# dominikh/jello

Hardware: AMD Instinct MI355X
Metric: Mpixels/sec fine-raster + paths/sec, 100k-path 4096^2 scene (higher is better)
Workload: dtype f32

## Files before the change

jello_amd/csrc/kernels_flatten.hip:

```cpp
#include <hip/hip_runtime.h>
__shared__ double fl_atan_tab[9];
#define JD_ATAN_TAB_LDS fl_atan_tab
#include "kcommon.h"
#define FF_INLINE __device__ __forceinline__
#include "flatten_fast.h"

using namespace jk;
using namespace jd;

namespace {

struct CubicParams { float th0, th1, chord_len, err; };
struct EulerParams { float th0, th1, k0, k1, ch; };
struct CubicPoints { V2 p0, p1, p2, p3; };
struct PointDeriv { V2 point, deriv; };
struct PathTagData { uint32_t tag_byte; MonoidK<5> monoid; };

#define DERIV_THRESH 1e-6f
#define DERIV_THRESH_SQUARED (DERIV_THRESH * DERIV_THRESH)
#define DERIV_EPS 1e-6f
#define SUBDIV_LIMIT (1.0f / 65536.0f)
#define K1_THRESH 1e-3f
#define DIST_THRESH 1e-3f
#define TANGENT_THRESH 1e-6f

#define FL_INVALID 0xffffffffu
#define FL_INFO_PIECE 0x80000000u
#define FL_INFO_DIRECT 0x40000000u
#ifndef FL_REFILL_LANES
#define FL_REFILL_LANES 32u
#endif

#define FL_MAX_REGIONS 8u
#define FL_MAX_GRAB 51200u
struct FlTemp {
    uint2* sinfo;
    uint4* recs;
    uint32_t* ctr;
    uint32_t K, R;
};
#define FL_CTR_CURSOR 512u
#define FL_CUR_STRIDE 64u
template <int KIND>
JD uint32_t fl_grab(const FlTemp& T, uint32_t home, uint32_t n, bool& failed) {
    uint32_t p = wave_bump(T.ctr + FL_CTR_CURSOR + FL_CUR_STRIDE * home + (KIND ? 32u : 0u), n);
    if (__builtin_expect(p <= T.R && n <= T.R - p, 1)) return home * T.R + p;
    failed = true;
    uint32_t region = home;
    for (uint32_t tries = 1u;; tries++) {
        if (KIND == 0 && p < T.R)
            for (uint32_t i = p; i < T.R; i++) T.sinfo[(size_t)region * T.R + i] = make_uint2(0u, 0u);
        if (p >= T.R) atomicSub(T.ctr + FL_CTR_CURSOR + FL_CUR_STRIDE * region + (KIND ? 32u : 0u), n);
        if (tries >= T.K) return FL_INVALID;
        region = region + 1u == T.K ? 0u : region + 1u;
        p = atomicAdd(T.ctr + FL_CTR_CURSOR + FL_CUR_STRIDE * region + (KIND ? 32u : 0u), n);
        if (p <= T.R && n <= T.R - p) return region * T.R + p;
    }
}
JD uint32_t fl_next_home(const FlTemp& T, uint32_t home, int kind) {
    uint32_t region = home;
    for (uint32_t tries = 0u; tries < T.K; tries++) {
        const uint32_t cur = __hip_atomic_load(T.ctr + FL_CTR_CURSOR + FL_CUR_STRIDE * region + (kind ? 32u : 0u), __ATOMIC_RELAXED, __HIP_MEMORY_SCOPE_AGENT);
        if (cur < T.R) return region;
        region = region + 1u == T.K ? 0u : region + 1u;
    }
    return home;
}

template <bool EMIT>
struct Out {
    const JlConfig* cfg;
    FlTemp T;
    uint32_t home_s, home_r;
    bool failed_s, failed_r;
    uint32_t slot;
    uint32_t cursor;
    uint32_t a_first, a_spos, a_rpos;

    JD uint32_t alloc(uint32_t n) {
        uint32_t first = cursor;
        cursor += n;
        if (EMIT) {
            a_first = first;
            a_spos = fl_grab<0>(T, home_s, n, failed_s);
            a_rpos = fl_grab<1>(T, home_r, n, failed_r);
        }
        return first;
    }
// ... 487 lines not shown
    }
}


JD V2 read_f32_point(const Scene& s, uint32_t ix) {
    uint32_t b = s.cfg->layout.pathdata_base + ix;
    return v2(u2f(s.scene.rd(b)), u2f(s.scene.rd(b + 1u)));
}
JD V2 read_i16_point(const Scene& s, uint32_t ix) {
    uint32_t raw = s.scene.rd(s.cfg->layout.pathdata_base + ix);
    float x = (float)((int32_t)(raw << 16) >> 16);
    float y = (float)((int32_t)raw >> 16);
    return v2(x, y);
}
JD PathTagData compute_tag_monoid(const Scene& s, uint32_t ix) {
    uint32_t tag_word = s.scene.rd(s.cfg->layout.pathtag_base + (ix >> 2));
    uint32_t shift = (ix & 3u) * 8u;
    MonoidK<5> tm = reduce_tag(tag_word & ((1u << shift) - 1u));
    JlTagMonoid pm = s.tag_monoids.rd(ix >> 2);
    tm.v[0] += pm.trans_ix; tm.v[1] += pm.pathseg_ix; tm.v[2] += pm.pathseg_offset; tm.v[3] += pm.style_ix; tm.v[4] += pm.path_ix;
    PathTagData r;
    r.tag_byte = (tag_word >> shift) & 0xffu;
    tm.v[0] -= 1u;
    tm.v[3] -= 2u;
    r.monoid = tm;
    return r;
}
JD CubicPoints read_path_segment(const Scene& s, const PathTagData& tag, bool is_stroke) {
    V2 p0 = v2(0, 0), p1 = v2(0, 0), p2 = v2(0, 0), p3 = v2(0, 0);
    uint32_t seg_type = tag.tag_byte & 3u;
    uint32_t pathseg_offset = tag.monoid.v[2];
    bool is_stroke_cap_marker = is_stroke && (tag.tag_byte & JL_PATH_TAG_SUBPATH_END) != 0u;
    bool is_open = seg_type == JL_PATH_TAG_QUADTO;
    if ((tag.tag_byte & JL_PATH_TAG_F32) != 0u) {
        p0 = read_f32_point(s, pathseg_offset);
        p1 = read_f32_point(s, pathseg_offset + 2u);
        if (seg_type >= JL_PATH_TAG_QUADTO) {
            p2 = read_f32_point(s, pathseg_offset + 4u);
            if (seg_type == JL_PATH_TAG_CUBICTO) p3 = read_f32_point(s, pathseg_offset + 6u);
        }
    } else {
        p0 = read_i16_point(s, pathseg_offset);
        p1 = read_i16_point(s, pathseg_offset + 1u);
        if (seg_type >= JL_PATH_TAG_QUADTO) {
            p2 = read_i16_point(s, pathseg_offset + 2u);
            if (seg_type == JL_PATH_TAG_CUBICTO) p3 = read_i16_point(s, pathseg_offset + 3u);
        }
    }
    if (is_stroke_cap_marker && is_open) {
        p0 = p1;
        p1 = p2;
        seg_type = JL_PATH_TAG_LINETO;
    }
    const float THIRD = (float)(1.0 / 3.0);
    if (seg_type == JL_PATH_TAG_LINETO) {
        p3 = p1;
        p2 = vmix(p3, p0, THIRD);
        p1 = vmix(p0, p3, THIRD);
    } else if (seg_type == JL_PATH_TAG_QUADTO) {
        p3 = p2;
        p2 = vmix(p1, p2, THIRD);
        p1 = vmix(p1, p0, THIRD);
    }
    CubicPoints r;
    r.p0 = p0; r.p1 = p1; r.p2 = p2; r.p3 = p3;
    return r;
}

struct Seg {
    PathTagData tag;
    uint32_t style_flags;
    bool is_stroke;
};

JD Seg load_seg(const Scene& s, uint32_t ix) {
    Seg r;
    r.tag = compute_tag_monoid(s, ix);
    r.style_flags = s.scene.rd(s.cfg->layout.style_base + r.tag.monoid.v[3]);
    r.is_stroke = (r.style_flags & JL_STYLE_FLAGS_STYLE) != 0u;
    return r;
}

#define FL_CTR_LIGHT 256u
#define FL_CTR_DEAL (FL_CTR_CURSOR + FL_CUR_STRIDE * FL_MAX_REGIONS)
#define FL_DEAL_GROUPS 256u
#define FL_DEAL_STRIDE 16u
#define FL_CTR_WORDS (FL_CTR_DEAL + FL_DEAL_STRIDE * FL_DEAL_GROUPS)
#ifndef PSC_BLOCKS
#define PSC_BLOCKS 2u
#endif
template <int SCAN>
__global__ __launch_bounds__(JL_WG) void k_flatten_classify(const JlConfig* __restrict__ cfg, Buf<uint32_t> scene, Buf<JlTagMonoid> reduced,
                                                                 Buf<JlTagMonoid> tag_monoids, uint32_t n_blocks, Buf<JlPathBbox> path_bboxes,
                                                                 uint32_t* __restrict__ list, uint32_t* __restrict__ counters, uint32_t cap,
                                                                 uint32_t n_tags, uint32_t* __restrict__ counts, uint32_t absorb,
                                                                 uint32_t* __restrict__ bump_words) {
    __shared__ uint32_t sh[20];
    __shared__ uint32_t sh_base[2];
    if (absorb & JH_ABSORB_BBOX_CLEAR) {
        const uint32_t n_clear = umin_(cfg->layout.n_path, path_bboxes.n);
        for (uint32_t i = blockIdx.x * JL_WG + threadIdx.x; i < n_clear; i += gridDim.x * JL_WG) {
            path_bboxes.p[i].x0 = 0x7fffffff;
            path_bboxes.p[i].y0 = 0x7fffffff;
            path_bboxes.p[i].x1 = (int32_t)0x80000000;
            path_bboxes.p[i].y1 = (int32_t)0x80000000;
        }
    }
    if ((absorb & JH_ABSORB_BUMP_CLEAR) && blockIdx.x == 0u && threadIdx.x < 8u) bump_words[threadIdx.x] = 0u;
    uint32_t nh[PSC_BLOCKS][4], nl[PSC_BLOCKS][4];
    uint32_t eh[PSC_BLOCKS], el[PSC_BLOCKS];
    uint32_t wg_h = 0u, wg_l = 0u;
#pragma unroll
    for (uint32_t blk = 0; blk < PSC_BLOCKS; blk++) {
        const uint32_t block = blockIdx.x * PSC_BLOCKS + blk;
        eh[blk] = 0u; el[blk] = 0u;
#pragma unroll
        for (uint32_t k = 0; k < 4u; k++) { nh[blk][k] = 0u; nl[blk][k] = 0u; }
        if (block >= n_blocks) continue;
        const uint32_t word_ix = block * JL_WG + threadIdx.x;
        const uint32_t tag_word = scene.rd(cfg->layout.pathtag_base + word_ix);
        MonoidK<5> pm;
        if (SCAN != 0) {
            MonoidK<5> prefix;
            if (SCAN == 1) prefix = parent_prefix(reduced, block, sh); else prefix = load_tm(reduced, block);
            MonoidK<5> tot5;
            if (SCAN == 1) __syncthreads();
            const MonoidK<5> ex = block_excl_scan_monoid<5>(reduce_tag(tag_word), sh, &tot5);
            pm = monoid_add(prefix, ex);
            if (tag_monoids.ok(word_ix)) {
                store_tm(&tag_monoids.p[word_ix], pm);
            } else {
#pragma unroll
                for (int i = 0; i < 5; i++) pm.v[i] = 0u;
            }
            __syncthreads();
        } else {
            pm = load_tm(tag_monoids, word_ix);
        }
        const uint32_t ix0 = word_ix * 4u;
        for (uint32_t q = 0u; q < 12u; q++) {
            const uint32_t sl = ix0 * 3u + q;
            if (sl < cap) counts[sl] = 0u;
        }
        uint32_t th = 0u, tl = 0u;
#pragma unroll
        for (uint32_t k = 0; k < 4u; k++) {
            const uint32_t ix = ix0 + k;
            if (ix >= n_tags) continue;
            const MonoidK<5> tm = monoid_add(pm, reduce_tag(tag_word & ((1u << (k * 8u)) - 1u)));
            const uint32_t tag_byte = (tag_word >> (k * 8u)) & 0xffu;
            const uint32_t style_flags = scene.rd(cfg->layout.style_base + tm.v[3] - 2u);
            const bool is_stroke = (style_flags & JL_STYLE_FLAGS_STYLE) != 0u;
            const uint32_t path_ix = tm.v[4];
            if ((tag_byte & JL_PATH_TAG_PATH) != 0u && path_bboxes.ok(path_ix)) {
                path_bboxes.p[path_ix].draw_flags = ((style_flags & JL_STYLE_FLAGS_FILL) == 0u) ? 0u : 1u;
                path_bboxes.p[path_ix].trans_ix = tm.v[0] - 1u;
            }
            const uint32_t seg_type = tag_byte & JL_PATH_TAG_SEG_TYPE;
            const bool curved = seg_type != JL_PATH_TAG_LINETO;
            if (seg_type != 0u) {
                if (!is_stroke) {
                    if (curved) nh[blk][k] = 1u; else nl[blk][k] = 1u;
                } else if ((tag_byte & JL_PATH_TAG_SUBPATH_END) != 0u) {
                    if (curved) nl[blk][k] = 1u;
                } else {
                    if (curved) { nh[blk][k] = 2u; nl[blk][k] = 1u; } else { nl[blk][k] = 3u; }
                }
            }
            th += nh[blk][k];
            tl += nl[blk][k];
        }
        MonoidK<2> m, tot;
        m.v[0] = th; m.v[1] = tl;
        const MonoidK<2> e2 = block_excl_scan_monoid<2>(m, sh, &tot);
        eh[blk] = wg_h + e2.v[0];
        el[blk] = wg_l + e2.v[1];
        wg_h += tot.v[0];
        wg_l += tot.v[1];
        __syncthreads();
    }
    if (threadIdx.x == 0) {
        sh_base[0] = wg_h ? atomicAdd(&counters[0], wg_h) : 0u;
        sh_base[1] = wg_l ? atomicAdd(&counters[FL_CTR_LIGHT], wg_l) : 0u;
    }
    __syncthreads();
#pragma unroll
    for (uint32_t blk = 0; blk < PSC_BLOCKS; blk++) {
        const uint32_t ix0 = ((blockIdx.x * PSC_BLOCKS + blk) * JL_WG + threadIdx.x) * 4u;
        uint32_t ph = sh_base[0] + eh[blk], pl = sh_base[1] + el[blk];
#pragma unroll
        for (uint32_t k = 0; k < 4u; k++) {
            const uint32_t ix = ix0 + k;
            uint32_t sub = 0u;
            for (uint32_t q = 0; q < nh[blk][k]; q++, sub++, ph++)
                if (ph < cap) list[ph] = ix * 3u + sub;
            for (uint32_t q = 0; q < nl[blk][k]; q++, sub++, pl++)
                if (pl < cap) list[cap - 1u - pl] = ix * 3u + sub;
        }
    }
}

template <bool EMIT>
JD void run_item(const JlConfig* cfg, const Scene& s, Out<EMIT>& o, uint32_t slot, EulerJob& job, uint32_t& path_ix_out) {
    uint32_t ix = slot / 3u, sub = slot - ix * 3u;
    Seg g = load_seg(s, ix);
    uint32_t path_ix = g.tag.monoid.v[4];
    path_ix_out = path_ix;
    uint32_t style_ix = g.tag.monoid.v[3];
    uint32_t trans_ix = g.tag.monoid.v[0];
    uint32_t style_flags = g.style_flags;
    job.path_ix = path_ix; job.trans_ix = trans_ix;
    Xf transform;
    {
        uint32_t base = cfg->layout.transform_base + trans_ix * 6u;
        transform.m0 = u2f(s.scene.rd(base)); transform.m1 = u2f(s.scene.rd(base + 1u)); transform.m2 = u2f(s.scene.rd(base + 2u));
        transform.m3 = u2f(s.scene.rd(base + 3u)); transform.t0 = u2f(s.scene.rd(base + 4u)); transform.t1 = u2f(s.scene.rd(base + 5u));
    }
    CubicPoints pts = read_path_segment(s, g.tag, g.is_stroke);
    if (g.is_stroke) {
        float linewidth = u2f(s.scene.rd(cfg->layout.style_base + style_ix + 1u));
        float offset = 0.5f * linewidth;
        bool is_stroke_cap_marker = (g.tag.tag_byte & JL_PATH_TAG_SUBPATH_END) != 0u;
        if (is_stroke_cap_marker) {
            V2 tangent = cubic_start_tangent(pts.p0, pts.p1, pts.p2, pts.p3);
            V2 offset_tangent = offset * normalize(tangent);
            V2 n = v2(offset_tangent.y * -1.0f, offset_tangent.x * 1.0f);
            draw_cap<EMIT>(o, path_ix, (style_flags & JL_STYLE_FLAGS_START_CAP_MASK) >> 2, pts.p0, pts.p0 - n, pts.p0 + n, -offset_tangent,
                           transform);
        } else {
            const float TT = TANGENT_THRESH * TANGENT_THRESH;
            V2 tan_prev = cubic_end_tangent(pts.p0, pts.p1, pts.p2, pts.p3);
            if (dot(tan_prev, tan_prev) < TT) tan_prev = v2(TANGENT_THRESH, 0.0f);
            V2 offset_tangent = offset * normalize(tan_prev);
            V2 n_prev = v2(offset_tangent.y * -1.0f, offset_tangent.x * 1.0f);
            if (sub < 2u) {
                V2 tan_start = cubic_start_tangent(pts.p0, pts.p1, pts.p2, pts.p3);
                if (dot(tan_start, tan_start) < TT) tan_start = v2(TANGENT_THRESH, 0.0f);
                V2 n_start = offset * normalize(v2(-tan_start.y, tan_start.x));
                job.valid = true; job.cubic = pts; job.local_to_device = transform;
                if (sub == 0u) { job.offset = offset; job.start_p = pts.p0 + n_start; job.end_p = pts.p3 + n_prev; }
                else { job.offset = -offset; job.start_p = pts.p0 - n_start; job.end_p = pts.p3 - n_prev; }
            } else {
                PathTagData ntag = compute_tag_monoid(s, ix + 1u);
                CubicPoints npts = read_path_segment(s, ntag, true);
                bool n_is_closed = (ntag.tag_byte & JL_PATH_TAG_SEG_TYPE) == JL_PATH_TAG_LINETO;
                bool n_is_marker = (ntag.tag_byte & JL_PATH_TAG_SUBPATH_END) != 0u;
                bool do_join = !n_is_marker || n_is_closed;
                if (do_join) {
                    V2 tan_next = cubic_start_tangent(npts.p0, npts.p1, npts.p2, npts.p3);
                    if (dot(tan_next, tan_next) < TT) tan_next = v2(TANGENT_THRESH, 0.0f);
                    V2 tnn = normalize(tan_next);
                    V2 n_next = v2((offset * tnn.y) * -1.0f, (offset * tnn.x) * 1.0f);
                    draw_join<EMIT>(o, path_ix, style_flags, pts.p3, tan_prev, tan_next, n_prev, n_next, transform);
                } else {
                    draw_cap<EMIT>(o, path_ix, (style_flags & JL_STYLE_FLAGS_END_CAP_MASK), pts.p3, pts.p3 + n_prev, pts.p3 - n_prev, offset_tangent,
                                   transform);
                }
            }
        }
    } else {
        job.valid = true; job.cubic = pts; job.local_to_device = transform;
        job.offset = 0.0f; job.start_p = pts.p0; job.end_p = pts.p3;
    }
}

#ifndef FLQ_STACK
#define FLQ_STACK 448u
#endif
#ifndef FLQ_LEAVES
#define FLQ_LEAVES 640u
#endif
#ifndef FLQ_MAX_LEVEL
#define FLQ_MAX_LEVEL 9u
#endif
struct FlBatch {
    uint32_t jhead[64];
    uint32_t stack[FLQ_STACK];
    uint32_t l_tpos[FLQ_LEAVES];
    uint16_t l_key[FLQ_LEAVES];
    uint16_t l_link[FLQ_LEAVES];
// ... 84 lines not shown
JD CubicParams piece_angles(const NodeEnds& ne) {
    const V2 chord = ne.point - ne.last_p;
    const float chord_squared = dot(chord, chord);
    CubicParams r;
    r.err = 0.0f;
    if (chord_squared < DERIV_THRESH_SQUARED) {
        r.th0 = 0.0f; r.th1 = 0.0f; r.chord_len = DERIV_THRESH;
        return r;
    }
    const V2 q0 = ne.last_q, q1 = ne.deriv;
    const V2 h0 = v2(q0.x * chord.x + q0.y * chord.y, q0.y * chord.x - q0.x * chord.y);
    const V2 h1 = v2(q1.x * chord.x + q1.y * chord.y, q1.x * chord.y - q1.y * chord.x);
    r.th0 = atan2_(h0.y, h0.x);
    r.th1 = atan2_(h1.y, h1.x);
    r.chord_len = sqrt_(chord_squared);
    return r;
}

struct PieceParams {
    EulerParams ep;
    float n, noff, int0, integral;
    uint32_t n_u, robust;
};
JD PieceParams piece_params(const CubicParams& cp, float scale, float offset) {
    const float tol = 0.25f;
    PieceParams r;
    r.ep = es_params_from_angles(cp.th0, cp.th1);
    const EulerParams& ep = r.ep;
    float k0 = ep.k0 - 0.5f * ep.k1;
    float k1 = ep.k1;
    float normalized_offset = offset / cp.chord_len;
    float dist_scaled = normalized_offset * ep.ch;
    float scale_multiplier = sqrt_(0.125f * scale * cp.chord_len / (ep.ch * tol));
    float a = 0.0f, b = 0.0f, integral = 0.0f, int0 = 0.0f, n_frac;
    uint32_t robust = 0u;
    if (abs_(k1) < K1_THRESH) {
        float k = ep.k0;
        n_frac = sqrt_(abs_(k * (k * dist_scaled + 1.0f)));
        robust = 1u;
    } else if (abs_(dist_scaled) < DIST_THRESH) {
        a = k1;
        b = k0;
        int0 = pow_1_5_signed(b);
        float int1 = pow_1_5_signed(a + b);
        integral = int1 - int0;
        n_frac = (float)(2.0 / 3.0) * integral / a;
        robust = 2u;
    } else {
        a = -2.0f * dist_scaled * k1;
        b = -1.0f - 2.0f * dist_scaled * k0;
        int0 = espc_int_approx(b);
        float int1 = espc_int_approx(a + b);
        integral = int1 - int0;
        float k_peak = k0 - k1 * b / a;
        float integrand_peak = sqrt_(abs_(k_peak * (k_peak * dist_scaled + 1.0f)));
        n_frac = integral * integrand_peak / a;
    }
    r.n = clamp_(ceil_(n_frac * scale_multiplier), 1.0f, 100.0f);
    r.n_u = to_u32(r.n);
    r.noff = normalized_offset;
    r.int0 = int0;
    r.integral = integral;
    r.robust = robust;
    return r;
}

#ifdef FL_FAST_CHECK
__device__ uint32_t g_ff_stats[8];
#endif
#ifndef FL_WAVES_PER_EU
#define FL_WAVES_PER_EU 4
#endif
#ifndef FL_BLOCKS_PER_CU
#define FL_BLOCKS_PER_CU 4
#endif
#ifdef FL_TIMING
#define FL_TL_WAVES 8192u
#define FL_TL_BATCHES 15u
#define FL_TL_WORDS (2u + 3u * FL_TL_BATCHES)
__device__ unsigned long long g_fl_timeline[FL_TL_WAVES * FL_TL_WORDS];
#endif
__global__ __launch_bounds__(JL_WG) __attribute__((amdgpu_waves_per_eu(FL_WAVES_PER_EU, FL_WAVES_PER_EU))) void k_flatten_items(const JlConfig* __restrict__ cfg, Buf<uint32_t> scene, Buf<JlTagMonoid> tag_monoids,
                                                         Buf<JlPathBbox> path_bboxes, const uint32_t* __restrict__ list,
                                                         uint32_t* __restrict__ counters, uint32_t cap, uint32_t* __restrict__ counts,
                                                         FlTemp T, uint32_t debug) {
    __shared__ FlBatch sh_batch[JL_WG / 64];
    Scene s;
    s.cfg = cfg; s.scene = scene; s.tag_monoids = tag_monoids;
    uint32_t n_heavy = umin_(counters[0], cap), n_light = umin_(counters[FL_CTR_LIGHT], cap - n_heavy);
    uint32_t n = n_heavy + n_light;
    const uint32_t units_h = n_heavy / 64u + (n_heavy % 64u != 0u ? 1u : 0u);
    const uint32_t units = units_h + n_light / 64u + (n_light % 64u != 0u ? 1u : 0u);
    const uint32_t n_groups = umin_(umax_(gridDim.x / FL_BLOCKS_PER_CU, 1u), FL_DEAL_GROUPS), group = blockIdx.x % n_groups;
    if (group >= units) return;
#ifdef FL_TIMING
    const unsigned long long tl_entry = wall_clock64();
    const uint32_t tl_wave = blockIdx.x * (JL_WG / 64u) + (threadIdx.x >> 6);
    uint32_t tl_n = 0u;
#endif
    atan_tab_fill();
    __syncthreads();
    const uint32_t lane = lane_id();
    FlBatch& B = sh_batch[threadIdx.x >> 6];
    Out<true> o;
    o.cfg = cfg; o.T = T; o.home_s = o.home_r = blockIdx.x % T.K; o.failed_s = o.failed_r = false; o.slot = 0u;
    if ((debug & 1u) != 0u) o.home_s = o.home_r = 0u;
#ifdef FL_SOAK_HOME0
    o.home_s = o.home_r = 0u;
#endif
    o.cursor = 0u; o.a_first = 0u; o.a_spos = 0u; o.a_rpos = 0u;
    for (;;) {
        uint32_t k = 0u;
        if (lane == 0u) k = atomicAdd(&counters[FL_CTR_DEAL + FL_DEAL_STRIDE * group], 1u);
        k = uni(k);
        const uint32_t u = k * n_groups + group;
        if (u >= units) break;
        const bool heavy = u < units_h;
        const uint32_t t_first = heavy ? u * 64u : n_heavy + (u - units_h) * 64u;
        const uint32_t t_end = umin_(t_first + 64u, heavy ? n_heavy : n);
        const uint32_t t = t_first + lane;
#ifdef FL_TIMING
        const unsigned long long tl_start = wall_clock64() | (heavy ? 1ull << 63 : 0ull);
        uint32_t tl_info = 0u;
#define FL_TL_END()                                                                                      \
    do {                                                                                                 \
        if (lane == 0u && tl_wave < FL_TL_WAVES && tl_n < FL_TL_BATCHES) {                               \
            g_fl_timeline[tl_wave * FL_TL_WORDS + 2u + 3u * tl_n] = tl_start;                            \
            g_fl_timeline[tl_wave * FL_TL_WORDS + 3u + 3u * tl_n] = wall_clock64();                      \
            g_fl_timeline[tl_wave * FL_TL_WORDS + 4u + 3u * tl_n] = tl_info;                             \
        }                                                                                                \
        tl_n++;                                                                                          \
    } while (0)
#else
#define FL_TL_END() do {} while (0)
#endif
        if (__builtin_amdgcn_ballot_w64(o.failed_s) != 0ull) { o.home_s = fl_next_home(T, o.home_s, 0); o.failed_s = false; }
        if (__builtin_amdgcn_ballot_w64(o.failed_r) != 0ull) { o.home_r = fl_next_home(T, o.home_r, 1); o.failed_r = false; }
        EulerJob job;
        job.valid = false; job.path_ix = 0u; job.trans_ix = 0u; job.offset = 0.0f;
        job.start_p = v2(0, 0); job.end_p = v2(0, 0);
        job.cubic.p0 = job.cubic.p1 = job.cubic.p2 = job.cubic.p3 = v2(0, 0);
        job.local_to_device = xf_identity();
        uint32_t slot = FL_INVALID;
        if (t < t_end) {
            slot = heavy ? list[t] : list[cap - 1u - (t - n_heavy)];
            o.slot = slot; o.cursor = 0u; o.a_first = 0u; o.a_spos = 0u; o.a_rpos = 0u;
            uint32_t path_ix;
            run_item<true>(cfg, s, o, slot, job, path_ix);
            if (!job.valid) counts[slot] = o.cursor;
        }
        EulerLane e;
        euler_begin(e, job);
        const bool active = job.valid && !e.done;
        if (__builtin_amdgcn_ballot_w64(active) == 0ull) {
            FL_TL_END();
            continue;
        }
        B.jhead[lane] = 0u;
        {
            const uint64_t am = __builtin_amdgcn_ballot_w64(active);
            if (active) B.stack[(uint32_t)__builtin_popcountll(am & ((1ull << lane) - 1ull))] = lane;
            if (lane == 0u) { B.n_stack = (uint32_t)__builtin_popcountll(am); B.n_leaves = 0u; B.bail = 0u; B.n_unsure = 0u; }
        }
        wave_sync();
#ifdef FL_SPLIT_NO_A
        if (lane == 0u) B.n_stack = 0u;
        wave_sync();
#endif
        for (;;) {
#ifdef FL_TIMING
            tl_info += 1u << 16;
#endif
            const uint32_t ns = uni(B.n_stack);
            const uint32_t nu = (uint32_t)__builtin_amdgcn_readfirstlane((int)B.n_unsure);
            if (ns == 0u && nu == 0u) break;
            const bool exact_round = ns == 0u || nu >= 64u;
            const uint32_t take = umin_(exact_round ? nu : ns, 64u);
            const bool has = lane < take;
            const uint32_t node = has ? (exact_round ? B.unsure[nu - 1u - lane] : B.stack[ns - 1u - lane]) : 0u;
            wave_sync();
            const uint32_t j = node & 63u, level = (node >> 6) & 31u, t0_u = node >> 11;
            const V2 jp0 = v2(read_lane_var(e.p0.x, j), read_lane_var(e.p0.y, j)), jp1 = v2(read_lane_var(e.p1.x, j), read_lane_var(e.p1.y, j));
            const V2 jp2 = v2(read_lane_var(e.p2.x, j), read_lane_var(e.p2.y, j)), jp3 = v2(read_lane_var(e.p3.x, j), read_lane_var(e.p3.y, j));
            const float scale = read_lane_var(e.scale, j);
            int kind = ffast::FF_UNSURE;
            if (exact_round) {
                if (has) kind = node_test(jp0, jp1, jp2, jp3, scale, level, t0_u).accept ? ffast::FF_ACCEPT : ffast::FF_REJECT;
            } else if (has) {
                float v_est, delta;
                kind = node_test_fast(jp0, jp1, jp2, jp3, scale, level, t0_u, &v_est, &delta);
#ifdef FL_FAST_CHECK
            }
            if (!exact_round) {
                bool c_unsure = false, c_contra = false, c_viol = false;
                if (has) {
                    float v2_, d2_;
                    const int k2 = node_test_fast(jp0, jp1, jp2, jp3, scale, level, t0_u, &v2_, &d2_);
                    const NodeResult rx = node_test(jp0, jp1, jp2, jp3, scale, level, t0_u);
                    const float vx = rx.cp.err * scale;
                    c_unsure = k2 == ffast::FF_UNSURE;
                    c_contra = (k2 == ffast::FF_ACCEPT && !rx.accept) || (k2 == ffast::FF_REJECT && rx.accept);
                    c_viol = (d2_ > 0.0f && !(abs_(v2_ - vx) <= d2_)) || (d2_ == 0.0f && k2 != ffast::FF_UNSURE && v2_ != 0.0f);
                }
                const uint32_t n0 = (uint32_t)__builtin_popcountll(__builtin_amdgcn_ballot_w64(has));
                const uint32_t n1 = (uint32_t)__builtin_popcountll(__builtin_amdgcn_ballot_w64(c_unsure));
                const uint32_t n2 = (uint32_t)__builtin_popcountll(__builtin_amdgcn_ballot_w64(c_contra));
                const uint32_t n3 = (uint32_t)__builtin_popcountll(__builtin_amdgcn_ballot_w64(c_viol));
                if (lane == 0u) {
                    atomicAdd(&g_ff_stats[0], n0);
                    if (n1) atomicAdd(&g_ff_stats[1], n1);
                    if (n2) atomicAdd(&g_ff_stats[2], n2);
                    if (n3) atomicAdd(&g_ff_stats[3], n3);
                }
#endif
            }
            const bool acc = has && kind == ffast::FF_ACCEPT, rej = has && kind == ffast::FF_REJECT, uns = has && kind == ffast::FF_UNSURE;
            const uint64_t accm = __builtin_amdgcn_ballot_w64(acc), rejm = __builtin_amdgcn_ballot_w64(rej), unsm = __builtin_amdgcn_ballot_w64(uns);
            const uint32_t n_acc = (uint32_t)__builtin_popcountll(accm), n_rej = (uint32_t)__builtin_popcountll(rejm);
            const uint32_t n_uns = (uint32_t)__builtin_popcountll(unsm);
            const uint32_t nl = uni(B.n_leaves);
            const uint32_t ns_left = exact_round ? ns : ns - take, nu_left = exact_round ? nu - take : nu;
            const bool too_deep = __builtin_amdgcn_ballot_w64(rej && level + 1u > FLQ_MAX_LEVEL) != 0ull;
            if (too_deep || ns_left + 2u * n_rej > FLQ_STACK || nl + n_acc > FLQ_LEAVES) {
                if (lane == 0u) B.bail = 1u;
                wave_sync();
                break;
            }
            const uint64_t below = (1ull << lane) - 1ull;
// ... 358 lines not shown
        const int32_t c = imax_(x1, dpp_move<CTRL, ROWS>(x1, x1)), d = imax_(y1, dpp_move<CTRL, ROWS>(y1, y1)); \
        if (take) { x0 = a; y0 = b; x1 = c; y1 = d; }                                        \
    }
            FB_SEG_STEP(JK_DPP_ROW_SHR(1), 0xf) FB_SEG_STEP(JK_DPP_ROW_SHR(2), 0xf) FB_SEG_STEP(JK_DPP_ROW_SHR(4), 0xf)
            FB_SEG_STEP(JK_DPP_ROW_SHR(8), 0xf) FB_SEG_STEP(JK_DPP_ROW_BCAST15, 0xa) FB_SEG_STEP(JK_DPP_ROW_BCAST31, 0xc)
#undef FB_SEG_STEP
            if (pix == c_path) {
                x0 = imin_(x0, cx0); y0 = imin_(y0, cy0); x1 = imax_(x1, cx1); y1 = imax_(y1, cy1);
            }
            const uint32_t pix_next = lane_next(pix, pix);
            if (valid && !skipped && pix_next != pix) fb_merge(path_bboxes, pix, x0, y0, x1, y1, pix == p_shared);
            c_path = (uint32_t)__builtin_amdgcn_readlane((int)pix, 63);
            cx0 = __builtin_amdgcn_readlane(x0, 63); cy0 = __builtin_amdgcn_readlane(y0, 63);
            cx1 = __builtin_amdgcn_readlane(x1, 63); cy1 = __builtin_amdgcn_readlane(y1, 63);
            if (ext) break;
        }
        if (c_path != FB_NONE && lane == 0u) fb_merge(path_bboxes, c_path, cx0, cy0, cx1, cy1, c_path == p_shared);
    }
}

}

#ifdef FL_FAST_CHECK
extern "C" int jh_debug_flatten_fast_stats(uint32_t* out8, int reset) {
    if (hipDeviceSynchronize() != hipSuccess) return -1;
    if (out8 && hipMemcpyFromSymbol(out8, HIP_SYMBOL(g_ff_stats), 8 * sizeof(uint32_t)) != hipSuccess) return -1;
    if (reset) {
        const uint32_t z[8] = {0, 0, 0, 0, 0, 0, 0, 0};
        if (hipMemcpyToSymbol(HIP_SYMBOL(g_ff_stats), z, sizeof z) != hipSuccess) return -1;
    }
    return 0;
}
#endif

#ifdef FL_TIMING
extern "C" int jh_debug_flatten_timeline(unsigned long long* out, uint32_t n_words, int reset, uint32_t* dims3) {
    if (hipDeviceSynchronize() != hipSuccess) return -1;
    if (dims3) {
        int dev = 0, khz = 0;
        if (hipGetDevice(&dev) != hipSuccess || hipDeviceGetAttribute(&khz, hipDeviceAttributeWallClockRate, dev) != hipSuccess) return -1;
        dims3[0] = FL_TL_WAVES; dims3[1] = FL_TL_WORDS; dims3[2] = (uint32_t)khz;
    }
    if (out) {
        if (n_words > FL_TL_WAVES * FL_TL_WORDS) return -1;
        if (hipMemcpyFromSymbol(out, HIP_SYMBOL(g_fl_timeline), (size_t)n_words * 8u) != hipSuccess) return -1;
    }
    if (reset) {
        void* p = nullptr;
        if (hipGetSymbolAddress(&p, HIP_SYMBOL(g_fl_timeline)) != hipSuccess) return -1;
        if (hipMemset(p, 0, sizeof(unsigned long long) * FL_TL_WAVES * FL_TL_WORDS) != hipSuccess) return -1;
    }
    return 0;
}
#endif

JhResult jh_launch_flatten(const JhLaunch& L) {
    if (L.gx == 0) return JH_L_OK;
    uint32_t n_tags = L.gx * JL_WG;
    uint64_t n_slots64 = (uint64_t)n_tags * 3;
    if (n_slots64 > 0xfffffff0ull) return JH_L_BAD_BINDINGS;
    uint32_t n_slots = (uint32_t)n_slots64;
    auto cfg = L.ptr<const JlConfig>(FL_CFG);
    auto scene = L.buf<uint32_t>(FL_SCENE);
    auto tm = L.buf<JlTagMonoid>(FL_TM);
    auto pb = L.buf<JlPathBbox>(FL_BBOX);
    JlBump* bump = L.ptr<JlBump>(FL_BUMP);
    auto lines = L.buf<JlLineSoup>(FL_LINES);
    uint32_t cap_blocks = L.cus() * FL_BLOCKS_PER_CU;
    uint32_t g = (n_slots + JL_WG - 1) / JL_WG;
    if (g > cap_blocks) g = cap_blocks;
    if ((L.debug_flatten & 8u) != 0u) g = 1u;
    const uint64_t line_cap = std::min<uint64_t>(std::max<uint64_t>(lines.n, 4096), 0xf0000000ull);
    FlTemp T;
    T.K = (uint32_t)std::min<uint64_t>(std::max<uint64_t>(line_cap >> 19, 1), FL_MAX_REGIONS);
    if ((L.debug_flatten & 2u) != 0u) T.K = FL_MAX_REGIONS;
#ifdef FL_SOAK_HOME0
    T.K = FL_MAX_REGIONS;
#endif
    T.R = (uint32_t)((line_cap + T.K - 1) / T.K) + FL_MAX_GRAB;
    const uint64_t tcap = (uint64_t)T.K * T.R;
    if (tcap > 0xfffffff0ull) return JH_L_BAD_BINDINGS;
    uint32_t* counts = (uint32_t*)jh_scratch_get(L.scratch, JH_SCR_A, (uint64_t)n_slots * 4);
    uint32_t* bases = (uint32_t*)jh_scratch_get(L.scratch, JH_SCR_B, (uint64_t)n_slots * 4);
    uint32_t* list = (uint32_t*)jh_scratch_get(L.scratch, JH_SCR_F, (uint64_t)n_slots * 4);
    T.sinfo = (uint2*)jh_scratch_get(L.scratch, JH_SCR_C, tcap * sizeof(uint2));
    T.recs = (uint4*)jh_scratch_get(L.scratch, JH_SCR_D, tcap * 64);
    if (!counts || !bases || !list || !T.sinfo || !T.recs) return JH_L_SCRATCH;
    uint32_t* counters = (uint32_t*)jh_scratch_acquire(L.scratch, JH_SCR_FL_CTR, FL_CTR_WORDS * 4, FL_CTR_WORDS * 4, L.stream);
    if (!counters) return JH_L_SCRATCH;
    T.ctr = counters;
    const JhAbsorbed& A = L.absorbed;
    const uint32_t absorb = (A.bbox_clear ? JH_ABSORB_BBOX_CLEAR : 0u) | (A.bump_clear ? JH_ABSORB_BUMP_CLEAR : 0u) | (A.pathtag_scan ? JH_ABSORB_PATHTAG_SCAN : 0u);
    {
        const uint32_t n_words = (n_tags + 3u) / 4u;
        uint32_t n_blocks = (n_words + JL_WG - 1u) / JL_WG;
        auto red = mkbuf<JlTagMonoid>(nullptr, 0);
        int scan = 0;
        if (A.pathtag_scan) {
            red = mkbuf<JlTagMonoid>(A.scan_reduced.ptr, A.scan_reduced.size);
            n_blocks = A.scan_wgs;
            scan = A.scan_small ? 1 : 2;
        }
        const dim3 gsc((n_blocks + PSC_BLOCKS - 1u) / PSC_BLOCKS);
        if (scan == 1)
            hipLaunchKernelGGL(k_flatten_classify<1>, gsc, dim3(JL_WG), 0, L.stream, cfg, scene, red, tm, n_blocks, pb, list, counters, n_slots, n_tags,
                               counts, absorb, (uint32_t*)bump);
        else if (scan == 2)
            hipLaunchKernelGGL(k_flatten_classify<2>, gsc, dim3(JL_WG), 0, L.stream, cfg, scene, red, tm, n_blocks, pb, list, counters, n_slots, n_tags,
                               counts, absorb, (uint32_t*)bump);
        else
            hipLaunchKernelGGL(k_flatten_classify<0>, gsc, dim3(JL_WG), 0, L.stream, cfg, scene, red, tm, n_blocks, pb, list, counters, n_slots, n_tags,
                               counts, absorb, (uint32_t*)bump);
    }
    hipLaunchKernelGGL(k_flatten_items, dim3(g), dim3(JL_WG), 0, L.stream, cfg, scene, tm, pb, (const uint32_t*)list, counters, n_slots, counts,
                       T, L.debug_flatten);
    JhResult rc = jh_scan_u32(L, counts, 1, bases, n_slots, nullptr, &bump->lines);
    if (rc) return rc;
    uint32_t gp = (uint32_t)((tcap + JL_WG - 1) / JL_WG);
    uint32_t gp_cap = L.cus() * 8u;
    uint32_t gl_cap = L.cus() * FL_LINES_WAVES_PER_EU;
    if (gp > gl_cap) gp = gl_cap;
    hipLaunchKernelGGL(k_flatten_lines, dim3(gp), dim3(JL_WG), 0, L.stream, cfg, scene, (const uint32_t*)counters, T, (const uint32_t*)bases, n_slots, lines);
    uint64_t gb64 = ((uint64_t)lines.n + 255u) / 256u;
#ifdef FB_MAX_BLOCKS
    const uint32_t gb_max = FB_MAX_BLOCKS;
#else
    const uint32_t gb_max = 4u * gp_cap;
#endif
    uint32_t gb = gb64 > gb_max ? gb_max : (uint32_t)(gb64 < 1u ? 1u : gb64);
    hipLaunchKernelGGL(k_flatten_bbox, dim3(gb), dim3(JL_WG), 0, L.stream, cfg, (const JlBump*)bump, (const uint32_t*)bases, n_slots, lines, pb,
                       counters, FL_CTR_WORDS);
    jh_scratch_left_clean(L.scratch, JH_SCR_FL_CTR);
    return JH_L_OK;
}
```

Baseline: 21460.

## Shard flatten work list across 16 sub-lists to spread atomic contention

The classify kernel now reserves list positions with atomics on one of 16 per-shard counter pairs, picked by workgroup index, instead of one global heavy and one global light counter. Each shard owns a fixed region of the list, filled heavy from the front and light from the back. The items kernel builds a per-wave prefix of unit counts over the 32 segments and maps each unit to its segment with a ballot and popcount. PSC_BLOCKS drops from 2 to 1 and the counts-zeroing store pattern becomes coalesced. The aim is less atomic serialization on two hot counters, at the cost of heavy items no longer being globally ordered before light ones and some extra per-unit lookup work.

```diff
diff --git a/jello_amd/csrc/flatten_sublists.h b/jello_amd/csrc/flatten_sublists.h
--- /dev/null
+++ b/jello_amd/csrc/flatten_sublists.h
@@ -0,0 +1,45 @@
+#pragma once
+#include <stdint.h>
+
+#ifndef FSL_INLINE
+#define FSL_INLINE static inline
+#endif
+
+#define FSL_MAX_SHARDS 16u
+#define FSL_UNIT 64u
+
+FSL_INLINE uint32_t fsl_shard_of_wg(uint32_t b, uint32_t K) { return b % K; }
+FSL_INLINE uint32_t fsl_wgs_of_shard(uint32_t G, uint32_t s, uint32_t K) { return G / K + (s < G % K ? 1u : 0u); }
+FSL_INLINE uint32_t fsl_shard_base(uint32_t G, uint32_t s, uint32_t K, uint32_t C) {
+    const uint32_t r = G % K;
+    return C * (s * (G / K) + (s < r ? s : r));
+}
+FSL_INLINE uint32_t fsl_shard_size(uint32_t G, uint32_t s, uint32_t K, uint32_t C) { return C * fsl_wgs_of_shard(G, s, K); }
+FSL_INLINE uint64_t fsl_total_entries(uint32_t G, uint32_t C) { return (uint64_t)C * G; }
+FSL_INLINE uint32_t fsl_heavy_pos(uint32_t base, uint32_t i) { return base + i; }
+FSL_INLINE uint32_t fsl_light_pos(uint32_t base, uint32_t size, uint32_t i) { return base + size - 1u - i; }
+FSL_INLINE uint32_t fsl_clamp_heavy(uint32_t counted_h, uint32_t size) { return counted_h < size ? counted_h : size; }
+FSL_INLINE uint32_t fsl_clamp_light(uint32_t counted_l, uint32_t n_heavy, uint32_t size) {
+    return counted_l < size - n_heavy ? counted_l : size - n_heavy;
+}
+FSL_INLINE uint32_t fsl_units_of(uint32_t n) { return n / FSL_UNIT + (n % FSL_UNIT != 0u ? 1u : 0u); }
+
+FSL_INLINE void fsl_unit_prefix(const uint32_t* n, uint32_t K, uint32_t* prefix) {
+    uint32_t sum = 0u;
+    for (uint32_t j = 0u; j < 2u * K; j++) {
+        prefix[j] = sum;
+        sum += fsl_units_of(n[j]);
+    }
+    prefix[2u * K] = sum;
+}
+FSL_INLINE bool fsl_segment_ends_by(uint32_t prefix_next, uint32_t u) { return prefix_next <= u; }
+FSL_INLINE uint32_t fsl_segment_of_unit(const uint32_t* prefix, uint32_t K, uint32_t u) {
+    uint32_t seg = 0u;
+    for (uint32_t j = 0u; j < 2u * K; j++) seg += fsl_segment_ends_by(prefix[j + 1u], u) ? 1u : 0u;
+    return seg;
+}
+FSL_INLINE void fsl_unit_items(uint32_t u, uint32_t seg_prefix, uint32_t seg_n, uint32_t* first, uint32_t* end) {
+    const uint32_t f = (u - seg_prefix) * FSL_UNIT;
+    *first = f;
+    *end = f + FSL_UNIT < seg_n ? f + FSL_UNIT : seg_n;
+}
diff --git a/jello_amd/csrc/kernels_flatten.hip b/jello_amd/csrc/kernels_flatten.hip
--- a/jello_amd/csrc/kernels_flatten.hip
+++ b/jello_amd/csrc/kernels_flatten.hip
@@ -4,6 +4,8 @@
 #include "kcommon.h"
 #define FF_INLINE __device__ __forceinline__
 #include "flatten_fast.h"
+#define FSL_INLINE __host__ __device__ __forceinline__
+#include "flatten_sublists.h"
 
 using namespace jk;
 using namespace jd;
@@ -657,13 +659,20 @@
 }
 
 #define FL_CTR_LIGHT 256u
+#ifndef FL_LIST_SHARDS
+#define FL_LIST_SHARDS 16u
+#endif
+#define FL_SHARD_STRIDE 16u
+static_assert(FL_LIST_SHARDS >= 1u && FL_LIST_SHARDS <= FSL_MAX_SHARDS && FL_LIST_SHARDS * FL_SHARD_STRIDE <= FL_CTR_LIGHT,
+              "the shards' counters lie in front of FL_CTR_LIGHT / FL_CTR_CURSOR");
 #define FL_CTR_DEAL (FL_CTR_CURSOR + FL_CUR_STRIDE * FL_MAX_REGIONS)
 #define FL_DEAL_GROUPS 256u
 #define FL_DEAL_STRIDE 16u
 #define FL_CTR_WORDS (FL_CTR_DEAL + FL_DEAL_STRIDE * FL_DEAL_GROUPS)
 #ifndef PSC_BLOCKS
-#define PSC_BLOCKS 2u
-#endif
+#define PSC_BLOCKS 1u
+#endif
+#define FL_WG_ITEMS (12u * PSC_BLOCKS * JL_WG)
 template <int SCAN>
 __global__ __launch_bounds__(JL_WG) void k_flatten_classify(const JlConfig* __restrict__ cfg, Buf<uint32_t> scene, Buf<JlTagMonoid> reduced,
                                                                  Buf<JlTagMonoid> tag_monoids, uint32_t n_blocks, Buf<JlPathBbox> path_bboxes,
@@ -714,7 +723,7 @@
         }
         const uint32_t ix0 = word_ix * 4u;
         for (uint32_t q = 0u; q < 12u; q++) {
-            const uint32_t sl = ix0 * 3u + q;
+            const uint32_t sl = block * (12u * JL_WG) + q * JL_WG + threadIdx.x;
             if (sl < cap) counts[sl] = 0u;
         }
         uint32_t th = 0u, tl = 0u;
@@ -754,11 +763,14 @@
         wg_l += tot.v[1];
         __syncthreads();
     }
+    const uint32_t shard = fsl_shard_of_wg(blockIdx.x, FL_LIST_SHARDS);
     if (threadIdx.x == 0) {
-        sh_base[0] = wg_h ? atomicAdd(&counters[0], wg_h) : 0u;
-        sh_base[1] = wg_l ? atomicAdd(&counters[FL_CTR_LIGHT], wg_l) : 0u;
+        sh_base[0] = wg_h ? atomicAdd(&counters[FL_SHARD_STRIDE * shard], wg_h) : 0u;
+        sh_base[1] = wg_l ? atomicAdd(&counters[FL_CTR_LIGHT + FL_SHARD_STRIDE * shard], wg_l) : 0u;
     }
     __syncthreads();
+    const uint32_t s_base = fsl_shard_base(gridDim.x, shard, FL_LIST_SHARDS, FL_WG_ITEMS);
+    const uint32_t s_size = fsl_shard_size(gridDim.x, shard, FL_LIST_SHARDS, FL_WG_ITEMS);
 #pragma unroll
     for (uint32_t blk = 0; blk < PSC_BLOCKS; blk++) {
         const uint32_t ix0 = ((blockIdx.x * PSC_BLOCKS + blk) * JL_WG + threadIdx.x) * 4u;
@@ -768,9 +780,9 @@
             const uint32_t ix = ix0 + k;
             uint32_t sub = 0u;
             for (uint32_t q = 0; q < nh[blk][k]; q++, sub++, ph++)
-                if (ph < cap) list[ph] = ix * 3u + sub;
+                if (ph < s_size) list[fsl_heavy_pos(s_base, ph)] = ix * 3u + sub;
             for (uint32_t q = 0; q < nl[blk][k]; q++, sub++, pl++)
-                if (pl < cap) list[cap - 1u - pl] = ix * 3u + sub;
+                if (pl < s_size) list[fsl_light_pos(s_base, s_size, pl)] = ix * 3u + sub;
         }
     }
 }
@@ -1021,15 +1033,27 @@
 #endif
 __global__ __launch_bounds__(JL_WG) __attribute__((amdgpu_waves_per_eu(FL_WAVES_PER_EU, FL_WAVES_PER_EU))) void k_flatten_items(const JlConfig* __restrict__ cfg, Buf<uint32_t> scene, Buf<JlTagMonoid> tag_monoids,
                                                          Buf<JlPathBbox> path_bboxes, const uint32_t* __restrict__ list,
-                                                         uint32_t* __restrict__ counters, uint32_t cap, uint32_t* __restrict__ counts,
+                                                         uint32_t* __restrict__ counters, uint32_t n_cls, uint32_t* __restrict__ counts,
                                                          FlTemp T, uint32_t debug) {
     __shared__ FlBatch sh_batch[JL_WG / 64];
+    __shared__ uint32_t sh_seg_n[2u * FL_LIST_SHARDS], sh_seg_prefix[2u * FL_LIST_SHARDS + 1u];
     Scene s;
     s.cfg = cfg; s.scene = scene; s.tag_monoids = tag_monoids;
-    uint32_t n_heavy = umin_(counters[0], cap), n_light = umin_(counters[FL_CTR_LIGHT], cap - n_heavy);
-    uint32_t n = n_heavy + n_light;
-    const uint32_t units_h = n_heavy / 64u + (n_heavy % 64u != 0u ? 1u : 0u);
-    const uint32_t units = units_h + n_light / 64u + (n_light % 64u != 0u ? 1u : 0u);
+    const uint32_t lane = lane_id();
+    uint32_t seg_n = 0u;
+    if (lane < 2u * FL_LIST_SHARDS) {
+        const uint32_t sh = lane < FL_LIST_SHARDS ? lane : lane - FL_LIST_SHARDS;
+        const uint32_t size = fsl_shard_size(n_cls, sh, FL_LIST_SHARDS, FL_WG_ITEMS);
+        const uint32_t nh = fsl_clamp_heavy(counters[FL_SHARD_STRIDE * sh], size);
+        seg_n = lane < FL_LIST_SHARDS ? nh : fsl_clamp_light(counters[FL_CTR_LIGHT + FL_SHARD_STRIDE * sh], nh, size);
+    }
+    const uint32_t seg_incl = wave_incl_scan_u32(fsl_units_of(seg_n));
+    const uint32_t units = read_lane(seg_incl, 63u);
+    if (threadIdx.x < 2u * FL_LIST_SHARDS) {
+        sh_seg_n[threadIdx.x] = seg_n;
+        sh_seg_prefix[threadIdx.x + 1u] = seg_incl;
+        if (threadIdx.x == 0u) sh_seg_prefix[0] = 0u;
+    }
     const uint32_t n_groups = umin_(umax_(gridDim.x / FL_BLOCKS_PER_CU, 1u), FL_DEAL_GROUPS), group = blockIdx.x % n_groups;
     if (group >= units) return;
 #ifdef FL_TIMING
@@ -1039,7 +1063,6 @@
 #endif
     atan_tab_fill();
     __syncthreads();
-    const uint32_t lane = lane_id();
     FlBatch& B = sh_batch[threadIdx.x >> 6];
     Out<true> o;
     o.cfg = cfg; o.T = T; o.home_s = o.home_r = blockIdx.x % T.K; o.failed_s = o.failed_r = false; o.slot = 0u;
@@ -1054,9 +1077,12 @@
         k = uni(k);
         const uint32_t u = k * n_groups + group;
         if (u >= units) break;
-        const bool heavy = u < units_h;
-        const uint32_t t_first = heavy ? u * 64u : n_heavy + (u - units_h) * 64u;
-        const uint32_t t_end = umin_(t_first + 64u, heavy ? n_heavy : n);
+        const bool seg_behind = lane < 2u * FL_LIST_SHARDS && fsl_segment_ends_by(sh_seg_prefix[lane + 1u], u);
+        const uint32_t seg = (uint32_t)__builtin_popcountll(__builtin_amdgcn_ballot_w64(seg_behind));
+        const bool heavy = seg < FL_LIST_SHARDS;
+        const uint32_t shard = heavy ? seg : seg - FL_LIST_SHARDS;
+        uint32_t t_first, t_end;
+        fsl_unit_items(u, sh_seg_prefix[seg], sh_seg_n[seg], &t_first, &t_end);
         const uint32_t t = t_first + lane;
 #ifdef FL_TIMING
         const unsigned long long tl_start = wall_clock64() | (heavy ? 1ull << 63 : 0ull);
@@ -1082,7 +1108,8 @@
         job.local_to_device = xf_identity();
         uint32_t slot = FL_INVALID;
         if (t < t_end) {
-            slot = heavy ? list[t] : list[cap - 1u - (t - n_heavy)];
+            const uint32_t s_base = fsl_shard_base(n_cls, shard, FL_LIST_SHARDS, FL_WG_ITEMS);
+            slot = list[heavy ? fsl_heavy_pos(s_base, t) : fsl_light_pos(s_base, fsl_shard_size(n_cls, shard, FL_LIST_SHARDS, FL_WG_ITEMS), t)];
             o.slot = slot; o.cursor = 0u; o.a_first = 0u; o.a_spos = 0u; o.a_rpos = 0u;
             uint32_t path_ix;
             run_item<true>(cfg, s, o, slot, job, path_ix);
@@ -1607,26 +1634,28 @@
     if (tcap > 0xfffffff0ull) return JH_L_BAD_BINDINGS;
     uint32_t* counts = (uint32_t*)jh_scratch_get(L.scratch, JH_SCR_A, (uint64_t)n_slots * 4);
     uint32_t* bases = (uint32_t*)jh_scratch_get(L.scratch, JH_SCR_B, (uint64_t)n_slots * 4);
-    uint32_t* list = (uint32_t*)jh_scratch_get(L.scratch, JH_SCR_F, (uint64_t)n_slots * 4);
+    const JhAbsorbed& A = L.absorbed;
+    const uint32_t n_words = (n_tags + 3u) / 4u;
+    const uint32_t n_blocks = A.pathtag_scan ? A.scan_wgs : (n_words + JL_WG - 1u) / JL_WG;
+    const uint32_t n_cls = (n_blocks + PSC_BLOCKS - 1u) / PSC_BLOCKS;
+    const uint64_t n_list = fsl_total_entries(n_cls, FL_WG_ITEMS);
+    if (n_list > 0xfffffff0ull) return JH_L_BAD_BINDINGS;
+    uint32_t* list = (uint32_t*)jh_scratch_get(L.scratch, JH_SCR_F, n_list * 4);
     T.sinfo = (uint2*)jh_scratch_get(L.scratch, JH_SCR_C, tcap * sizeof(uint2));
     T.recs = (uint4*)jh_scratch_get(L.scratch, JH_SCR_D, tcap * 64);
     if (!counts || !bases || !list || !T.sinfo || !T.recs) return JH_L_SCRATCH;
     uint32_t* counters = (uint32_t*)jh_scratch_acquire(L.scratch, JH_SCR_FL_CTR, FL_CTR_WORDS * 4, FL_CTR_WORDS * 4, L.stream);
     if (!counters) return JH_L_SCRATCH;
     T.ctr = counters;
-    const JhAbsorbed& A = L.absorbed;
     const uint32_t absorb = (A.bbox_clear ? JH_ABSORB_BBOX_CLEAR : 0u) | (A.bump_clear ? JH_ABSORB_BUMP_CLEAR : 0u) | (A.pathtag_scan ? JH_ABSORB_PATHTAG_SCAN : 0u);
     {
-        const uint32_t n_words = (n_tags + 3u) / 4u;
-        uint32_t n_blocks = (n_words + JL_WG - 1u) / JL_WG;
         auto red = mkbuf<JlTagMonoid>(nullptr, 0);
         int scan = 0;
         if (A.pathtag_scan) {
             red = mkbuf<JlTagMonoid>(A.scan_reduced.ptr, A.scan_reduced.size);
-            n_blocks = A.scan_wgs;
             scan = A.scan_small ? 1 : 2;
         }
-        const dim3 gsc((n_blocks + PSC_BLOCKS - 1u) / PSC_BLOCKS);
+        const dim3 gsc(n_cls);
         if (scan == 1)
             hipLaunchKernelGGL(k_flatten_classify<1>, gsc, dim3(JL_WG), 0, L.stream, cfg, scene, red, tm, n_blocks, pb, list, counters, n_slots, n_tags,
                                counts, absorb, (uint32_t*)bump);
@@ -1637,7 +1666,7 @@
             hipLaunchKernelGGL(k_flatten_classify<0>, gsc, dim3(JL_WG), 0, L.stream, cfg, scene, red, tm, n_blocks, pb, list, counters, n_slots, n_tags,
                                counts, absorb, (uint32_t*)bump);
     }
-    hipLaunchKernelGGL(k_flatten_items, dim3(g), dim3(JL_WG), 0, L.stream, cfg, scene, tm, pb, (const uint32_t*)list, counters, n_slots, counts,
+    hipLaunchKernelGGL(k_flatten_items, dim3(g), dim3(JL_WG), 0, L.stream, cfg, scene, tm, pb, (const uint32_t*)list, counters, n_cls, counts,
                        T, L.debug_flatten);
     JhResult rc = jh_scan_u32(L, counts, 1, bases, n_slots, nullptr, &bump->lines);
     if (rc) return rc;
```

Measured after the change: 21550, median of 6. Within noise of the previous version (+0.4%).
